# Samirez/Visual_odometry

Measured on AMD Instinct MI355X. Metric: frame-pairs/sec (1280x720, 2000 ORB feats), higher is better.
Workload: dtype u8+f32+f64; 1 GPU; seeded synthetic 1280x720 drone flight (256 distinct rendered views, closed loop), 2000 ORB features/frame, 8 levels = BASELINE config 2; chunk of 257 consecutive frames -> 256 pairs (k, k+1) per GPU per step, each frame detected once; detector=orb, distinct_rendered_frames=256, pair_stride=1, contexts_per_gpu=3, keypoint_order=cv2, poly_solver=fast, matcher=crosscheck, matcher_kernel=mfma_fp4, ransac=5-point, conf 0.99, 1 px, seed 2^64-1, <=1000 iters, parallelism=single GPU, pairs_ok_last_step=256

## Files before the change

visual_odometry_amd/csrc/geom_kernels.hip:

```cpp
#include "vo_internal.h"
#include "chain_common.h"
#include <float.h>

#define WAVE 64
#ifndef VO_DK_FAST_CAP
#define VO_DK_FAST_CAP 64
#endif
#ifndef VO_DK_ITERS
#define VO_DK_ITERS 300
#endif

__device__ __forceinline__ double vo_hypot(double a, double b)
{
    a = fabs(a); b = fabs(b);
    if (a < b) { double t = a; a = b; b = t; }
    if (a == 0) return 0;
    double r = b / a;
    return a * sqrt(1 + r * r);
}

template <int M, int N>
__device__ __forceinline__ void jacobi_svd(double* At, double* W, double* Vt)
{
    const double eps = DBL_EPSILON * 10;
// ... 98 lines not shown
{
    PolyTab t{};
    for (int i = 0; i < 4; i++)
        for (int j = 0; j < 4; j++) {
            int a = k_e1[i][0] + k_e1[j][0], b = k_e1[i][1] + k_e1[j][1], c = k_e1[i][2] + k_e1[j][2];
            int idx = -1;
            for (int m = 0; m < 10; m++) if (k_e2[m][0] == a && k_e2[m][1] == b && k_e2[m][2] == c) idx = m;
            t.t11[i][j] = idx;
        }
    for (int i = 0; i < 10; i++)
        for (int j = 0; j < 4; j++) {
            int a = k_e2[i][0] + k_e1[j][0], b = k_e2[i][1] + k_e1[j][1], c = k_e2[i][2] + k_e1[j][2];
            int idx = -1;
            for (int m = 0; m < 20; m++) if (k_e3[m][0] == a && k_e3[m][1] == b && k_e3[m][2] == c) idx = m;
            t.t21[i][j] = idx;
        }
    return t;
}

__device__ __forceinline__ void mul11_acc(const double* p, const double* q, double s, double* r)
{
    constexpr PolyTab T = make_poly_tab();
#pragma unroll
    for (int i = 0; i < 4; i++)
#pragma unroll
        for (int j = 0; j < 4; j++) r[T.t11[i][j]] += s * p[i] * q[j];
}

__device__ __forceinline__ void mul21_acc(const double* p, const double* q, double s, double* r)
{
    constexpr PolyTab T = make_poly_tab();
#pragma unroll
    for (int i = 0; i < 10; i++)
#pragma unroll
        for (int j = 0; j < 4; j++) r[T.t21[i][j]] += s * p[i] * q[j];
}

struct cplx { double re, im; };
__device__ __forceinline__ cplx cmul(cplx a, cplx b) { return {a.re * b.re - a.im * b.im, a.re * b.im + a.im * b.re}; }
__device__ __forceinline__ cplx cdiv(cplx a, cplx b)
{
    double t = 1. / (b.re * b.re + b.im * b.im);
    return {(a.re * b.re + a.im * b.im) * t, (-a.re * b.im + a.im * b.re) * t};
}

template <int NA, int NB>
__device__ __forceinline__ void conv(const double* a, const double* b, double* r)
{
#pragma unroll
    for (int i = 0; i <= NA + NB; i++) r[i] = 0;
#pragma unroll
    for (int i = 0; i <= NA; i++)
#pragma unroll
        for (int j = 0; j <= NB; j++) r[i + j] += a[i] * b[j];
}

template <int O>
__device__ __forceinline__ int quad_bcast(int v) { return __builtin_amdgcn_mov_dpp(v, O * 0x55, 0xf, 0xf, true); }
template <int O>
__device__ __forceinline__ double quad_bcast(double v)
{
    const int lo = quad_bcast<O>(__double2loint(v)), hi = quad_bcast<O>(__double2hiint(v));
    return __hiloint2double(hi, lo);
}
__device__ __forceinline__ double quad_bcast_from(int o, double v)
{
    switch (o) {
    case 0: return quad_bcast<0>(v);
    case 1: return quad_bcast<1>(v);
    case 2: return quad_bcast<2>(v);
    default: return quad_bcast<3>(v);
    }
}
__device__ __forceinline__ double sel4(int q, double a, double b, double c, double d) { return q == 0 ? a : q == 1 ? b : q == 2 ? c : d; }

__device__ __forceinline__ bool dk_exit(double max_diff, double max_mag, bool conv_all, bool early, double& prev, int& stall)
{
    if (max_diff <= 0 || (early && conv_all)) return true;
    const double small = 1e-7 * (1.0 + max_mag);
    if (early && max_diff < small * small) {
        if (max_diff > 0.25 * prev) { if (++stall >= 2) return true; }
        else stall = 0;
    }
    prev = max_diff;
    return false;
}

__device__ __forceinline__ void dk_iterate_quad(const double* c, double* rr, double* ri, bool early, int q)
{
    double prev = 1e300;
    int stall = 0;
    const int sweeps = early ? VO_DK_FAST_CAP : VO_DK_ITERS;
#pragma unroll 1
    for (int iter = 0; iter < sweeps; iter++) {
        bool conv_all = true;
        double max_diff = 0, max_mag = 0;
        double pr[3], pi[3], nr[3], ni[3], dr[3], di[3];
#pragma unroll
        for (int t = 0; t < 2; t++) {
            pr[t] = sel4(q, rr[4 * t], rr[4 * t + 1], rr[4 * t + 2], rr[4 * t + 3]);
            pi[t] = sel4(q, ri[4 * t], ri[4 * t + 1], ri[4 * t + 2], ri[4 * t + 3]);
        }
        pr[2] = (q & 1) ? rr[9] : rr[8]; pi[2] = (q & 1) ? ri[9] : ri[8];
#pragma unroll
        for (int t = 0; t < 3; t++) { nr[t] = c[10]; ni[t] = 0; dr[t] = c[10]; di[t] = 0; }
#pragma unroll
        for (int j = 0; j < 10; j++)
#pragma unroll
            for (int t = 0; t < 3; t++) {
                const cplx np = cmul({nr[t], ni[t]}, {pr[t], pi[t]});
                nr[t] = np.re + c[9 - j]; ni[t] = np.im;
            }
#pragma unroll
        for (int i = 0; i < 10; i++) {
            const int t = i >> 2, o = i & 3;
            cplx denom = {dr[t], di[t]};
#pragma unroll
            for (int j = i + 1; j < 10; j++) denom = cmul(denom, {pr[t] - rr[j], pi[t] - ri[j]});
            const bool coincident = q == o && !(fabs(denom.re) > 0) && !(fabs(denom.im) > 0);
            if (__any(coincident)) {
                if (coincident) {
                    denom = {c[10], 0};
#pragma unroll
                    for (int j = 0; j < 10; j++)
                        if (j != i) {
                            const cplx d = {rr[i] - rr[j], ri[i] - ri[j]};
                            if (d.re != 0 || d.im != 0) denom = cmul(denom, d);
                        }
                }
            }
            cplx num = cdiv({nr[t], ni[t]}, denom);
            num.re = quad_bcast_from(o, num.re); num.im = quad_bcast_from(o, num.im);
            rr[i] = rr[i] - num.re; ri[i] = ri[i] - num.im;
            const double ab2 = num.re * num.re + num.im * num.im;
            max_diff = fmax(max_diff, ab2);
            const double mag = fabs(rr[i]) + fabs(ri[i]);
            max_mag = fmax(max_mag, mag);
            const double lim = 4 * DBL_EPSILON * mag;
            conv_all &= ab2 <= lim * lim;
#pragma unroll
            for (int t2 = t; t2 < 3; t2++) {
                if (t2 == t && o == 3) continue;
                const cplx m = cmul({dr[t2], di[t2]}, {pr[t2] - rr[i], pi[t2] - ri[i]});
                const bool mine = t2 > t || q > o;
                dr[t2] = mine ? m.re : dr[t2]; di[t2] = mine ? m.im : di[t2];
            }
        }
        if (dk_exit(max_diff, max_mag, conv_all, early, prev, stall)) break;
    }
}

__device__ __forceinline__ void dk_iterate_low(const double* c, int n, double* rr, double* ri, bool early)
{
    double prev = 1e300;
    int stall = 0;
    const int sweeps = early ? VO_DK_FAST_CAP : VO_DK_ITERS;
#pragma unroll 1
    for (int iter = 0; iter < sweeps; iter++) {
        bool conv_all = true;
        double max_diff = 0, max_mag = 0;
#pragma unroll
        for (int i = 0; i < 10; i++) {
            if (i < n) {
                cplx p = {rr[i], ri[i]};
                double lead = c[10];
#pragma unroll
                for (int q = 1; q <= 10; q++) if (q == n) lead = c[q];
                cplx num = {lead, 0}, denom = {lead, 0};
#pragma unroll
                for (int j = 0; j < 10; j++) {
                    if (j < n) {
                        double cj = c[9 - j];
#pragma unroll
                        for (int q = 0; q < 10; q++) if (q == n - j - 1) cj = c[q];
                        cplx np = cmul(num, p);
                        num.re = np.re + cj; num.im = np.im;
                        if (j != i) {
                            cplx d = {p.re - rr[j], p.im - ri[j]};
                            if (d.re != 0 || d.im != 0) denom = cmul(denom, d);
                        }
                    }
                }
                num = cdiv(num, denom);
                rr[i] = p.re - num.re; ri[i] = p.im - num.im;
                const double ab2 = num.re * num.re + num.im * num.im;
                max_diff = fmax(max_diff, ab2);
                const double mag = fabs(rr[i]) + fabs(ri[i]);
                max_mag = fmax(max_mag, mag);
                const double lim = 4 * DBL_EPSILON * mag;
                conv_all &= ab2 <= lim * lim;
            }
        }
        if (dk_exit(max_diff, max_mag, conv_all, early, prev, stall)) break;
    }
}

#define FP_QUADS 16
typedef __attribute__((address_space(3))) double lds_double;
#define CMQ(r, j) cm[((r) * 5 + (j)) * 64 + lane]
#define CMK(r, k) cm[((r) * 5 + (k) % 5) * 64 + (lane & ~3) + (k) / 5]
__device__ __forceinline__ void quad_lds_sync()
{
    __builtin_amdgcn_fence(__ATOMIC_RELEASE, "wavefront");
    __builtin_amdgcn_wave_barrier();
    __builtin_amdgcn_fence(__ATOMIC_ACQUIRE, "wavefront");
}

__device__ __noinline__ int five_point_solve_quad(const double* x1, const double* x2, double* Eout, lds_double* cm, bool dk_early)
{
    const int lane = threadIdx.x & 63, q = lane & 3;
    double basis[36];
    {
        double A[9][5], V[5][9];
#pragma unroll
        for (int i = 0; i < 5; i++) {
            double u1 = x1[2 * i], v1 = x1[2 * i + 1], u2 = x2[2 * i], v2 = x2[2 * i + 1];
            A[0][i] = u2 * u1; A[1][i] = u2 * v1; A[2][i] = u2;
            A[3][i] = v2 * u1; A[4][i] = v2 * v1; A[5][i] = v2;
            A[6][i] = u1; A[7][i] = v1; A[8][i] = 1.0;
        }
        bool bad = false;
#pragma unroll
        for (int k = 0; k < 5; k++) {
            double nrm = 0;
#pragma unroll
            for (int r = k; r < 9; r++) nrm += A[r][k] * A[r][k];
            nrm = sqrt(nrm);
            bad |= nrm < 1e-300;
            double alpha = A[k][k] > 0 ? -nrm : nrm;
#pragma unroll
            for (int r = 0; r < 9; r++) V[k][r] = r < k ? 0.0 : A[r][k];
            V[k][k] -= alpha;
            double vn = 0;
#pragma unroll
            for (int r = k; r < 9; r++) vn += V[k][r] * V[k][r];
            vn = sqrt(vn);
            bad |= vn < 1e-300;
#pragma unroll
            for (int r = k; r < 9; r++) V[k][r] /= vn;
#pragma unroll
            for (int c = k; c < 5; c++) {
                double d = 0;
#pragma unroll
                for (int r = k; r < 9; r++) d += V[k][r] * A[r][c];
#pragma unroll
                for (int r = k; r < 9; r++) A[r][c] -= 2 * d * V[k][r];
            }
        }
        if (bad) return 0;
#pragma unroll
        for (int j = 0; j < 4; j++) {
            double e[9];
#pragma unroll
            for (int r = 0; r < 9; r++) e[r] = (r == 5 + j) ? 1.0 : 0.0;
#pragma unroll
            for (int k = 4; k >= 0; k--) {
                double d = 0;
#pragma unroll
                for (int r = k; r < 9; r++) d += V[k][r] * e[r];
#pragma unroll
                for (int r = k; r < 9; r++) e[r] -= 2 * d * V[k][r];
            }
#pragma unroll
            for (int r = 0; r < 9; r++) basis[j * 9 + r] = e[r];
        }
    }

    {
        double E[3][3][4];
#pragma unroll
        for (int r = 0; r < 3; r++)
#pragma unroll
            for (int c = 0; c < 3; c++)
#pragma unroll
                for (int k = 0; k < 4; k++) E[r][c][k] = basis[k * 9 + r * 3 + c];
        {
            double row[20];
#pragma unroll
            for (int i = 0; i < 20; i++) row[i] = 0;
#pragma unroll
            for (int c = 0; c < 3; c++) {
                const int c1 = (c + 1) % 3, c2 = (c + 2) % 3;
                double m[10];
#pragma unroll
                for (int i = 0; i < 10; i++) m[i] = 0;
                mul11_acc(E[1][c1], E[2][c2], 1.0, m);
                mul11_acc(E[1][c2], E[2][c1], -1.0, m);
                mul21_acc(m, E[0][c], 1.0, row);
            }
#pragma unroll
            for (int j = 0; j < 5; j++) CMQ(0, j) = sel4(q, row[j], row[5 + j], row[10 + j], row[15 + j]);
        }
        double L[3][3][10];
#pragma unroll
        for (int r = 0; r < 3; r++)
#pragma unroll
            for (int c = 0; c < 3; c++) {
#pragma unroll
                for (int i = 0; i < 10; i++) L[r][c][i] = 0;
#pragma unroll
                for (int k = 0; k < 3; k++) mul11_acc(E[r][k], E[c][k], 1.0, L[r][c]);
            }
        double tr[10];
#pragma unroll
        for (int i = 0; i < 10; i++) tr[i] = L[0][0][i] + L[1][1][i] + L[2][2][i];
#pragma unroll
        for (int r = 0; r < 3; r++)
#pragma unroll
            for (int i = 0; i < 10; i++) L[r][r][i] -= 0.5 * tr[i];
#pragma unroll
        for (int r = 0; r < 3; r++)
#pragma unroll
            for (int c = 0; c < 3; c++) {
                double row[20];
#pragma unroll
                for (int i = 0; i < 20; i++) row[i] = 0;
#pragma unroll
                for (int k = 0; k < 3; k++) mul21_acc(L[r][k], E[k][c], 1.0, row);
#pragma unroll
                for (int j = 0; j < 5; j++) CMQ(1 + r * 3 + c, j) = sel4(q, row[j], row[5 + j], row[10 + j], row[15 + j]);
            }
    }
    quad_lds_sync();

#pragma unroll 1
    for (int col = 0; col < 10; col++) {
        int piv = col;
        double best = fabs(CMK(col, col));
#pragma unroll 1
        for (int r = col + 1; r < 10; r++) { double v = fabs(CMK(r, col)); if (v > best) { best = v; piv = r; } }
        if (best < 1e-300) return 0;
        double prow[5], f[10];
        const double inv = 1.0 / CMK(piv, col);
        quad_lds_sync();
#pragma unroll
        for (int j = 0; j < 5; j++) {
            const double a = CMQ(piv, j), b = CMQ(col, j);
            prow[j] = a * inv;
            CMQ(piv, j) = b;
            CMQ(col, j) = prow[j];
        }
        quad_lds_sync();
#pragma unroll
        for (int r = 0; r < 10; r++) f[r] = CMK(r, col);
        quad_lds_sync();
#pragma unroll
        for (int r = 0; r < 10; r++) {
            if (r == col || f[r] == 0) continue;
#pragma unroll
            for (int j = 0; j < 5; j++) CMQ(r, j) -= f[r] * prow[j];
        }
        quad_lds_sync();
    }

    double Bx[3][4], By[3][4], Bc[3][5];
#pragma unroll
    for (int i = 0; i < 3; i++) {
        double r1[10], r2[10];
#pragma unroll
        for (int k = 0; k < 10; k++) { r1[k] = CMK(2 * i + 4, 10 + k); r2[k] = CMK(2 * i + 5, 10 + k); }
        Bx[i][3] = -r2[0]; Bx[i][2] = r1[0] - r2[1]; Bx[i][1] = r1[1] - r2[2]; Bx[i][0] = r1[2];
        By[i][3] = -r2[3]; By[i][2] = r1[3] - r2[4]; By[i][1] = r1[4] - r2[5]; By[i][0] = r1[5];
        Bc[i][4] = -r2[6]; Bc[i][3] = r1[6] - r2[7]; Bc[i][2] = r1[7] - r2[8]; Bc[i][1] = r1[8] - r2[9]; Bc[i][0] = r1[9];
    }
    double c[11];
    {
        double t1[8], t2[8], t3[11];
#pragma unroll
        for (int i = 0; i < 11; i++) c[i] = 0;
        conv<3, 4>(By[1], Bc[2], t1); conv<3, 4>(By[2], Bc[1], t2);
#pragma unroll
        for (int i = 0; i < 8; i++) t1[i] -= t2[i];
        conv<3, 7>(Bx[0], t1, t3);
#pragma unroll
        for (int i = 0; i < 11; i++) c[i] += t3[i];
        conv<3, 4>(Bx[1], Bc[2], t1); conv<3, 4>(Bx[2], Bc[1], t2);
#pragma unroll
        for (int i = 0; i < 8; i++) t1[i] -= t2[i];
        conv<3, 7>(By[0], t1, t3);
#pragma unroll
        for (int i = 0; i < 11; i++) c[i] -= t3[i];
        conv<3, 3>(Bx[1], By[2], t1); conv<3, 3>(Bx[2], By[1], t2);
#pragma unroll
        for (int i = 0; i < 7; i++) t1[i] -= t2[i];
        conv<4, 6>(Bc[0], t1, t3);
#pragma unroll
        for (int i = 0; i < 11; i++) c[i] += t3[i];
    }

    int n = 10;
    while (n > 1 && !(fabs(c[n]) > DBL_EPSILON)) n--;
    double rr[10], ri[10];
    {
        cplx p = {1, 0}, r = {1, 1};
#pragma unroll
        for (int i = 0; i < 10; i++) { rr[i] = p.re; ri[i] = p.im; p = cmul(p, r); }
    }
    if (n == 10) dk_iterate_quad(c, rr, ri, dk_early, q);
    else dk_iterate_low(c, n, rr, ri, dk_early);

    uint32_t real_mask = 0;
#pragma unroll
    for (int k = 0; k < 10; k++) {
        double zi = ri[k];
        if (fabs(zi) < 1e-100) zi = 0;
        if (k < n && !(fabs(zi) > 1e-10)) real_mask |= 1u << k;
    }
    const int nreal = __popc(real_mask);
    int count = 0;
#pragma unroll 1
    for (int m0 = 0; m0 < nreal; m0 += 4) {
        const int m = m0 + q;
        double zr = 0;
        {
            int ord = 0;
#pragma unroll
            for (int k = 0; k < 10; k++) {
                const bool set = (real_mask >> k) & 1;
                if (set && ord == m) zr = rr[k];
                ord += set;
            }
        }
        double en[9];
#pragma unroll
        for (int k = 0; k < 9; k++) en[k] = 0;
        int keep = 0;
        if (m < nreal) {
            double z1 = zr, z2 = z1 * z1, z3 = z2 * z1, z4 = z3 * z1;
            double bz[9], xy1[3];
#pragma unroll
            for (int j = 0; j < 3; j++) {
                bz[j * 3 + 0] = Bx[j][3] * z3 + Bx[j][2] * z2 + Bx[j][1] * z1 + Bx[j][0];
                bz[j * 3 + 1] = By[j][3] * z3 + By[j][2] * z2 + By[j][1] * z1 + By[j][0];
                bz[j * 3 + 2] = Bc[j][4] * z4 + Bc[j][3] * z3 + Bc[j][2] * z2 + Bc[j][1] * z1 + Bc[j][0];
            }
            solve_z<3>(bz, xy1);
            if (!(fabs(xy1[2]) < 1e-10)) {
                double x = xy1[0] / xy1[2], y = xy1[1] / xy1[2], nrm = 0, e[9];
#pragma unroll
                for (int k = 0; k < 9; k++) {
                    e[k] = basis[k] * x + basis[9 + k] * y + basis[18 + k] * z1 + basis[27 + k];
                    nrm += e[k] * e[k];
                }
                nrm = sqrt(nrm);
#pragma unroll
                for (int k = 0; k < 9; k++) en[k] = e[k] / nrm;
                keep = 1;
            }
        }
#define FP_STORE_MODEL(o)                                                                             \
        if (quad_bcast<o>(keep)) {                                                                    \
            double w[9];                                                                              \
            _Pragma("unroll") for (int k = 0; k < 9; k++) w[k] = quad_bcast<o>(en[k]);                \
            double* dst = Eout + count * 9;                                                           \
            dst[q] = sel4(q, w[0], w[1], w[2], w[3]);                                                 \
            dst[4 + q] = sel4(q, w[4], w[5], w[6], w[7]);                                             \
            dst[8] = w[8];                                                                            \
            count++;                                                                                  \
        }
        FP_STORE_MODEL(0) FP_STORE_MODEL(1) FP_STORE_MODEL(2) FP_STORE_MODEL(3)
#undef FP_STORE_MODEL
    }
    return count;
}

__device__ __forceinline__ uint32_t rng_next(uint64_t& state)
{
    state = (uint64_t)(uint32_t)state * 4164903690ULL + (uint32_t)(state >> 32);
    return (uint32_t)state;
}

__device__ int ransac_update_num_iters(double p, double ep, int model_points, int max_iters)
{
    p = fmax(p, 0.); p = fmin(p, 1.);
    ep = fmax(ep, 0.); ep = fmin(ep, 1.);
    double num = fmax(1. - p, DBL_MIN);
    double denom = 1. - pow(1. - ep, (double)model_points);
    if (denom < DBL_MIN) return 0;
    num = log(num);
    denom = log(denom);
    return (denom >= 0 || -num >= max_iters * (-denom)) ? max_iters : __double2int_rn(num / denom);
}

__device__ __forceinline__ float sampson_err(const double* E, double u1, double v1, double u2, double v2)
{
    double Ex0 = E[0] * u1 + E[1] * v1 + E[2], Ex1 = E[3] * u1 + E[4] * v1 + E[5], Ex2 = E[6] * u1 + E[7] * v1 + E[8];
    double Et0 = E[0] * u2 + E[3] * v2 + E[6], Et1 = E[1] * u2 + E[4] * v2 + E[7];
    double d = u2 * Ex0 + v2 * Ex1 + Ex2;
    return (float)(d * d / (Ex0 * Ex0 + Ex1 * Ex1 + Et0 * Et0 + Et1 * Et1));
}

__device__ __forceinline__ int count_inliers(const double* E, const double* x1, const double* x2, int M, float t,
                                             int lane, int stride, int first, uint8_t* mask_out)
{
    int good = 0;
    for (int base = first; base < M; base += stride) {
        const int i = base + lane;
        bool f = false;
        if (i < M) {
            f = sampson_err(E, x1[2 * i], x1[2 * i + 1], x2[2 * i], x2[2 * i + 1]) <= t;
            if (mask_out) mask_out[i] = f ? 1 : 0;
        }
        good += __popcll(__ballot(f));
    }
    return good;
}

#define RS_STREAM 512
#define RS_SCORE_G 4
#ifndef RS_WAVES
#define RS_WAVES 4
#endif
#ifndef RS_SOLVERS
#define RS_SOLVERS 4
#endif
#define RS_ROUND (FP_QUADS * RS_SOLVERS)
#define RS_THREADS (64 * RS_WAVES)
static_assert(RS_SOLVERS >= 1 && RS_SOLVERS <= RS_WAVES && RS_ROUND <= 64, "the sampler and the model list hold at most 64 samples per round");

struct RansacShared {
    double cm[200 * RS_ROUND];
    uint32_t stream[RS_STREAM];
    int sub[64][5];
    int nm[64];
    int off[65];
    uint8_t eh[640];
    int cnt[RS_WAVES * RS_SCORE_G];
    int used;
};

__global__ __launch_bounds__(RS_THREADS, 1) void k_ransac(PairBuf pb, int kp_cap, RansacParams rp, const uint32_t* rng_tab, int rng_n)
{
    extern __shared__ __attribute__((aligned(16))) unsigned char s_dyn[];
    RansacShared& sh = *(RansacShared*)s_dyn;
    const int p = blockIdx.x, tid = threadIdx.x, lane = tid & 63, wave = tid >> 6;
    const int M = pb.m_count[p];
    const double* x1 = pb.xn1 + (size_t)p * kp_cap * 2;
    const double* x2 = pb.xn2 + (size_t)p * kp_cap * 2;
    uint8_t* mask = pb.mask + (size_t)p * kp_cap;
    vo_pair_result* res = pb.res + p;

    if (M < 5) {
        if (tid == 0) { res->status = VO_ERR_TOO_FEW; res->n_inl = 0; res->ransac_iters = 0; }
        for (int i = tid; i < M; i += RS_THREADS) mask[i] = 0;
        return;
    }
    const double threshold = rp.thresh_px / ((rp.K[0] + rp.K[4]) / 2);
    const float t = (float)(threshold * threshold);

    if (M == 5) {
        if (tid < 4) {
            double* models = pb.models + (size_t)p * 64 * 90;
            const int nm = five_point_solve_quad(x1, x2, models, (lds_double*)sh.cm, rp.dk_early != 0);
            __threadfence_block();
            if (tid == 0) {
                for (int k = 0; k < 9; k++) res->E[k] = nm > 0 ? models[k] : 0.0;
                res->status = nm > 0 ? VO_OK : VO_ERR_NO_MODEL;
                res->n_inl = nm > 0 ? 5 : 0;
                res->reserved = nm;
                res->ransac_iters = 0;
            }
        }
        if (tid < 5) mask[tid] = 1;
        return;
    }

    int niters = rp.max_iters > 1 ? rp.max_iters : 1;
    int max_good = 0, iters_done = 0, pos = 0;
    double bestE[9];
#pragma unroll
    for (int k = 0; k < 9; k++) bestE[k] = 0;

#ifdef VO_EXP_TIMING
    long long tA = clock64(), tB = 0, tC = 0, tD = 0, tE = 0;
#endif
    double* gmodels = pb.models + (size_t)p * 64 * 90;
    for (int r0 = 0; r0 < niters; r0 += RS_ROUND) {
        const int nh = min(RS_ROUND, niters - r0);
        for (int i = tid; i < RS_STREAM; i += RS_THREADS) sh.stream[i] = pos + i < rng_n ? rng_tab[pos + i] % (uint32_t)M : 0u;
        __syncthreads();
        if (wave == 0) {
            int start = 5 * lane, used = 5;
            for (;;) {
                int idx[5];
                used = 0;
                if (lane < nh) {
#pragma unroll
                    for (int i = 0; i < 5; i++) {
                        int v; bool dup;
                        do {
                            const int at = start + used;
                            if (at < RS_STREAM && pos + at < rng_n) v = (int)sh.stream[at];
                            else {
                                uint64_t st = rp.seed ? rp.seed : 0xffffffffULL;
                                uint32_t x = 0;
                                if (pos + at < rng_n) x = rng_tab[pos + at];
                                else { for (int q = 0; q <= pos + at; q++) x = rng_next(st); }
                                v = (int)(x % (uint32_t)M);
                            }
                            used++;
                            dup = false;
#pragma unroll
                            for (int k = 0; k < 5; k++) dup |= k < i && idx[k] == v;
                        } while (dup);
                        idx[i] = v;
                    }
#pragma unroll
                    for (int i = 0; i < 5; i++) sh.sub[lane][i] = idx[i];
                }
                int inc = used;
#pragma unroll
                for (int d = 1; d < 64; d <<= 1) { const int o = __shfl_up(inc, d, 64); if (lane >= d) inc += o; }
                const int true_start = inc - used;
                const bool moved = lane < nh && true_start != start;
                start = true_start;
                if (lane == 63) sh.used = inc;
                if (!__any(moved)) break;
            }
        }
        __syncthreads();
        pos += sh.used;
#ifdef VO_EXP_TIMING
        if (r0 == 0) tB = clock64();
#endif
        if (wave < RS_SOLVERS) {
            const int h = wave * FP_QUADS + (lane >> 2);
            if (h < nh) {
                double s1[10], s2[10];
#pragma unroll
                for (int i = 0; i < 5; i++) {
                    const int v = sh.sub[h][i];
                    s1[2 * i] = x1[2 * v]; s1[2 * i + 1] = x1[2 * v + 1];
                    s2[2 * i] = x2[2 * v]; s2[2 * i + 1] = x2[2 * v + 1];
                }
                const int nm = five_point_solve_quad(s1, s2, gmodels + h * 90, (lds_double*)sh.cm + wave * (200 * FP_QUADS), rp.dk_early != 0);
                if ((lane & 3) == 0) sh.nm[h] = nm;
            }
        }
        __syncthreads();
        if (wave == 0) {
            const int nm = lane < nh ? sh.nm[lane] : 0;
            int inc = nm;
#pragma unroll
            for (int d = 1; d < 64; d <<= 1) { int v = __shfl_up(inc, d, 64); if (lane >= d) inc += v; }
            sh.off[lane] = inc - nm;
            if (lane == 63) sh.off[64] = inc;
            for (int m = 0; m < nm; m++) sh.eh[inc - nm + m] = (uint8_t)lane;
        }
        __syncthreads();
#ifdef VO_EXP_TIMING
        if (r0 == 0) tC = clock64();
#endif
        const int T = sh.off[64];
        bool done = false;
        int last_h = -1;
        for (int b0 = 0; b0 < T && !done; b0 += RS_WAVES * RS_SCORE_G) {
            {
                double E[RS_SCORE_G][9];
                int ne = 0;
#pragma unroll
                for (int gq = 0; gq < RS_SCORE_G; gq++) {
                    const int e = b0 + gq * RS_WAVES + wave;
                    const int ee = e < T ? e : (b0 + wave < T ? b0 + wave : 0);
                    const int h = sh.eh[ee], m = ee - sh.off[h];
#pragma unroll
                    for (int k = 0; k < 9; k++) E[gq][k] = gmodels[h * 90 + m * 9 + k];
                    ne += e < T;
                }
                if (ne > 0) {
                    int good[RS_SCORE_G];
#pragma unroll
                    for (int gq = 0; gq < RS_SCORE_G; gq++) good[gq] = 0;
                    for (int base = 0; base < M; base += 64) {
                        const int i = base + lane;
                        const bool in = i < M;
                        const double u1 = in ? x1[2 * i] : 0.0, v1 = in ? x1[2 * i + 1] : 0.0, u2 = in ? x2[2 * i] : 0.0, v2 = in ? x2[2 * i + 1] : 0.0;
#pragma unroll
                        for (int gq = 0; gq < RS_SCORE_G; gq++)
                            good[gq] += (int)__popcll(__ballot(in && sampson_err(E[gq], u1, v1, u2, v2) <= t));
                    }
                    if (lane == 0) {
#pragma unroll
                        for (int gq = 0; gq < RS_SCORE_G; gq++) sh.cnt[gq * RS_WAVES + wave] = good[gq];
                    }
                }
            }
            __syncthreads();
            for (int q = 0; q < RS_WAVES * RS_SCORE_G; q++) {
                const int e2 = b0 + q;
                if (e2 >= T) break;
                const int h = sh.eh[e2];
                if (h != last_h) {
                    if (r0 + h >= niters) { done = true; break; }
                    last_h = h;
                    iters_done = r0 + h + 1;
                }
                const int good = sh.cnt[q];
                if (good > max(max_good, 4)) {
                    const int m = e2 - sh.off[h];
#pragma unroll
                    for (int k = 0; k < 9; k++) bestE[k] = gmodels[h * 90 + m * 9 + k];
                    max_good = good;
                    niters = ransac_update_num_iters(rp.prob, (double)(M - good) / M, 5, niters);
                }
            }
            __syncthreads();
        }
        if (!done) iters_done = min(r0 + nh, niters);
        __syncthreads();
#ifdef VO_EXP_TIMING
        if (r0 == 0) tD = clock64();
#endif
    }

    if (max_good > 0) {
        count_inliers(bestE, x1, x2, M, t, tid, RS_THREADS, 0, mask);
        if (tid == 0) {
#pragma unroll
            for (int k = 0; k < 9; k++) res->E[k] = bestE[k];
            res->n_inl = max_good; res->status = VO_OK; res->ransac_iters = iters_done; res->reserved = 1;
#ifdef VO_EXP_TIMING
            tE = clock64();
            res->n_kp1 = (int)(tB - tA); res->n_kp2 = (int)(tC - tB); res->n_match = (int)(tD - tC); res->n_good = (int)(tE - tD); res->reserved = iters_done;
#endif
        }
    } else {
        for (int i = tid; i < M; i += RS_THREADS) mask[i] = 0;
        if (tid == 0) { res->n_inl = 0; res->status = VO_ERR_NO_MODEL; res->ransac_iters = iters_done; res->reserved = 0; }
    }
}

void launch_ransac(hipStream_t s, PairBuf pb, int kp_cap, int P, RansacParams rp, const uint32_t* rng_tab, int rng_n)
{
    static bool attr = false;
    if (!attr) { (void)hipFuncSetAttribute((const void*)k_ransac, hipFuncAttributeMaxDynamicSharedMemorySize, (int)sizeof(RansacShared)); attr = true; }
    hipLaunchKernelGGL(k_ransac, dim3(P), dim3(RS_THREADS), sizeof(RansacShared), s, pb, kp_cap, rp, rng_tab, rng_n);
}

__device__ __forceinline__ void triangulate_one(const double* P1, const double* P2, double x1, double y1,
                                                double x2, double y2, double* X)
{
    double A[16];
#pragma unroll
    for (int k = 0; k < 4; k++) {
        A[0 * 4 + k] = x1 * P1[8 + k] - P1[k];
        A[1 * 4 + k] = y1 * P1[8 + k] - P1[4 + k];
        A[2 * 4 + k] = x2 * P2[8 + k] - P2[k];
        A[3 * 4 + k] = y2 * P2[8 + k] - P2[4 + k];
    }
    solve_z<4>(A, X);
}

__global__ void k_triangulate_raw(const double* P1g, const double* P2g, const double* x1, const double* x2,
                                  int M, double* X)
{
    int i = blockIdx.x * blockDim.x + threadIdx.x;
    if (i >= M) return;
    double P1[12], P2[12], q[4];
#pragma unroll
    for (int k = 0; k < 12; k++) { P1[k] = P1g[k]; P2[k] = P2g[k]; }
    triangulate_one(P1, P2, x1[i], x1[M + i], x2[i], x2[M + i], q);
#pragma unroll
    for (int k = 0; k < 4; k++) X[(size_t)k * M + i] = q[k];
}

void launch_triangulate_raw(hipStream_t s, const double* P1, const double* P2, const double* x1, const double* x2,
                            int M, double* X)
{
    if (M <= 0) return;
    hipLaunchKernelGGL(k_triangulate_raw, dim3((M + 63) / 64), dim3(64), 0, s, P1, P2, x1, x2, M, X);
}

__global__ void k_triangulate_pairs(PairBuf pb, int kp_cap, RansacParams rp)
{
    const int p = blockIdx.y;
    const vo_pair_result* res = pb.res + p;
    if (res->status != VO_OK) return;
    int i = blockIdx.x * blockDim.x + threadIdx.x;
    if (i >= res->n_inl) return;
    const double* R = res->R; const double* t = res->t; const double* K = rp.K;
    double T[12], P[12], P0[12];
#pragma unroll
    for (int r = 0; r < 3; r++) {
#pragma unroll
        for (int c = 0; c < 3; c++) T[r * 4 + c] = R[c * 3 + r];
        T[r * 4 + 3] = -(R[0 * 3 + r] * t[0] + R[1 * 3 + r] * t[1] + R[2 * 3 + r] * t[2]);
    }
#pragma unroll
// ... 76 lines not shown
{
    double Q[4];
    triangulate_one(P0, P, a[0], a[1], b[0], b[1], Q);
    const double w = Q[2] * Q[3];
    const double q0 = Q[0] / Q[3], q1 = Q[1] / Q[3], q2 = Q[2] / Q[3], q3 = Q[3] / Q[3];
    const double z = P[8] * q0 + P[9] * q1 + P[10] * q2 + P[11] * q3;
    pos = w > 0 && q2 < dist && z > 0 && z < dist;
    neg = w < 0 && -q2 < dist && -z > 0 && -z < dist;
}

__global__ __launch_bounds__(256) void k_pose_prepare(PairBuf pb, int kp_cap)
{
    __shared__ int s_w[4];
    const int p = blockIdx.x, tid = threadIdx.x, lane = tid & 63, wave = tid >> 6;
    vo_pair_result* res = pb.res + p;
    PoseState* ps = pb.pose_state + p;
    if (res->status != VO_OK) {
        if (tid == 0) { res->n_good = 0; ps->active = 0; }
        return;
    }
    if (res->reserved != 1) {
        __syncthreads();
        if (tid == 0) { res->status = VO_ERR_AMBIGUOUS; res->n_good = 0; ps->active = 0; }
        return;
    }
    const int M = pb.m_count[p];
    const size_t base2 = (size_t)p * kp_cap * 2;
    const uint8_t* mask = pb.mask + (size_t)p * kp_cap;
    double* in1 = pb.in1 + base2; double* in2 = pb.in2 + base2;
    double* ip1 = pb.ipx1 + base2; double* ip2 = pb.ipx2 + base2;
    int ninl = 0;
    for (int b = 0; b < M; b += 256) {
        const int i = b + tid;
        const bool f = i < M && mask[i] != 0;
        const unsigned long long bal = __ballot(f);
        __syncthreads();
        if (lane == 0) s_w[wave] = __popcll(bal);
        __syncthreads();
        int off = 0, tot = 0;
#pragma unroll
        for (int w = 0; w < 4; w++) { const int c = s_w[w]; if (w < wave) off += c; tot += c; }
        if (f) {
            const int pos = ninl + off + __popcll(bal & ((1ULL << lane) - 1));
            in1[2 * pos] = pb.xn1[base2 + 2 * i]; in1[2 * pos + 1] = pb.xn1[base2 + 2 * i + 1];
            in2[2 * pos] = pb.xn2[base2 + 2 * i]; in2[2 * pos + 1] = pb.xn2[base2 + 2 * i + 1];
            ip1[2 * pos] = pb.px1[base2 + 2 * i]; ip1[2 * pos + 1] = pb.px1[base2 + 2 * i + 1];
            ip2[2 * pos] = pb.px2[base2 + 2 * i]; ip2[2 * pos + 1] = pb.px2[base2 + 2 * i + 1];
        }
        ninl += tot;
    }
    if (tid < 64) {
        double E[9], R1[9], R2[9], tt[3];
#pragma unroll
        for (int k = 0; k < 9; k++) E[k] = res->E[k];
        decompose_essential(E, R1, R2, tt);
        if (tid == 0) {
#pragma unroll
            for (int k = 0; k < 9; k++) { ps->R1[k] = R1[k]; ps->R2[k] = R2[k]; }
#pragma unroll
            for (int k = 0; k < 3; k++) ps->t[k] = tt[k];
#pragma unroll
            for (int k = 0; k < 4; k++) ps->good[k] = 0;
            ps->ninl = ninl; ps->active = 1;
        }
    }
}

__device__ __forceinline__ void pose_candidate(const PoseState* ps, int c, double* P)
{
    const double* Rc = c ? ps->R2 : ps->R1;
#pragma unroll
    for (int r = 0; r < 3; r++) {
#pragma unroll
        for (int k = 0; k < 3; k++) P[r * 4 + k] = Rc[r * 3 + k];
        P[r * 4 + 3] = ps->t[r];
    }
}

__global__ __launch_bounds__(256) void k_pose(PairBuf pb, int kp_cap, RansacParams rp)
{
    const int p = blockIdx.x, blk = blockIdx.y, c = blockIdx.z, lane = threadIdx.x & 63;
    PoseState* ps = pb.pose_state + p;
    if (!ps->active) return;
    const int ninl = ps->ninl, i = blk * 256 + threadIdx.x;
    if (blk * 256 >= ninl) return;
    const size_t base2 = (size_t)p * kp_cap * 2;
    const double* in1 = pb.in1 + base2; const double* in2 = pb.in2 + base2;
    const double P0[12] = {1, 0, 0, 0, 0, 1, 0, 0, 0, 0, 1, 0};
    double P[12];
    pose_candidate(ps, c, P);
    bool mp = false, mn = false;
    if (i < ninl) cheirality2(P0, P, in1 + 2 * i, in2 + 2 * i, rp.dist_thresh, mp, mn);
    const int gp = __popcll(__ballot(mp)), gn = __popcll(__ballot(mn));
    if (lane == 0 && gp) atomicAdd(&ps->good[c], gp);
    if (lane == 0 && gn) atomicAdd(&ps->good[c + 2], gn);
}

__global__ __launch_bounds__(256) void k_pose_finish(PairBuf pb, int kp_cap, RansacParams rp)
{
    const int p = blockIdx.x;
    const PoseState* ps = pb.pose_state + p;
    if (!ps->active) return;
    vo_pair_result* res = pb.res + p;
    const int ninl = ps->ninl;
    const int g0 = ps->good[0], g1 = ps->good[1], g2 = ps->good[2], g3 = ps->good[3];
    int best;
    if (g0 >= g1 && g0 >= g2 && g0 >= g3) best = 0;
    else if (g1 >= g0 && g1 >= g2 && g1 >= g3) best = 1;
    else if (g2 >= g0 && g2 >= g1 && g2 >= g3) best = 2;
    else best = 3;
    if (pb.pose_mask) {
        const size_t base2 = (size_t)p * kp_cap * 2;
        const double* in1 = pb.in1 + base2; const double* in2 = pb.in2 + base2;
        const double P0[12] = {1, 0, 0, 0, 0, 1, 0, 0, 0, 0, 1, 0};
        double P[12];
        pose_candidate(ps, best & 1, P);
        uint8_t* pm = pb.pose_mask + (size_t)p * kp_cap;
        for (int i = threadIdx.x; i < ninl; i += blockDim.x) {
            bool mp, mn;
            cheirality2(P0, P, in1 + 2 * i, in2 + 2 * i, rp.dist_thresh, mp, mn);
            pm[i] = (best >= 2 ? mn : mp) ? 255 : 0;
        }
    }
    if (threadIdx.x == 0) {
        const double* Rb = (best & 1) ? ps->R2 : ps->R1;
#pragma unroll
        for (int k = 0; k < 9; k++) res->R[k] = Rb[k];
#pragma unroll
        for (int k = 0; k < 3; k++) res->t[k] = best >= 2 ? -ps->t[k] : ps->t[k];
        res->n_good = best == 0 ? g0 : best == 1 ? g1 : best == 2 ? g2 : g3;
        res->n_inl = ninl;
    }
}

void launch_pose(hipStream_t s, PairBuf pb, int kp_cap, int P, RansacParams rp)
{
    hipLaunchKernelGGL(k_pose_prepare, dim3(P), dim3(256), 0, s, pb, kp_cap);
    hipLaunchKernelGGL(k_pose, dim3(P, (kp_cap + 255) / 256, 2), dim3(256), 0, s, pb, kp_cap, rp);
    hipLaunchKernelGGL(k_pose_finish, dim3(P), dim3(pb.pose_mask ? 256 : 64), 0, s, pb, kp_cap, rp);
}

__global__ __launch_bounds__(64) void k_five_point_raw(const double* x1, const double* x2, double* E, int* nm, int dk_early)
{
    extern __shared__ __attribute__((aligned(16))) unsigned char s_dyn[];
    if (threadIdx.x < 4 && blockIdx.x == 0) {
        const int n = five_point_solve_quad(x1, x2, E, (lds_double*)s_dyn, dk_early != 0);
        if (threadIdx.x == 0) *nm = n;
    }
}

void launch_five_point_raw(hipStream_t s, const double* x1, const double* x2, double* E, int* nm, int dk_early)
{
    static bool attr = false;
    if (!attr) { (void)hipFuncSetAttribute((const void*)k_five_point_raw, hipFuncAttributeMaxDynamicSharedMemorySize, (int)(200 * FP_QUADS * sizeof(double))); attr = true; }
    hipLaunchKernelGGL(k_five_point_raw, dim3(1), dim3(64), 200 * FP_QUADS * sizeof(double), s, x1, x2, E, nm, dk_early);
}

__global__ void k_reprojection(const double* poses, int ncam, const double* points, int npt, const int* obs_cam,
                               const int* obs_pt, const double* obs_xy, int nobs, const double* Kd, double threshold,
                               double* sqerr, uint8_t* keep, int* bad)
{
    const int i = blockIdx.x * blockDim.x + threadIdx.x;
    if (i >= nobs) return;
    const int ci = obs_cam[i], pi = obs_pt[i];
    if (ci < 0 || ci >= ncam || pi < 0 || pi >= npt) { atomicOr(bad, 1); sqerr[i] = 0; keep[i] = 0; return; }
    const double e = reprojection_sqerr_one(poses + 16 * (size_t)ci, points + 3 * (size_t)pi, Kd, obs_xy[2 * i], obs_xy[2 * i + 1]);
    sqerr[i] = e;
    keep[i] = e < threshold ? 1 : 0;
}

void launch_reprojection(hipStream_t s, const double* poses, int ncam, const double* points, int npt, const int* obs_cam,
                         const int* obs_pt, const double* obs_xy, int nobs, const double* Kd, double threshold,
                         double* sqerr, uint8_t* keep, int* bad)
{
    if (nobs <= 0) return;
    hipLaunchKernelGGL(k_reprojection, dim3((nobs + 255) / 256), dim3(256), 0, s, poses, ncam, points, npt, obs_cam, obs_pt,
                       obs_xy, nobs, Kd, threshold, sqerr, keep, bad);
}

__global__ void k_track_link(const int* pair_frames, const int* match_off, const int* mq, const int* mt, int P, int cap,
                             unsigned long long* parent)
{
    const int p = blockIdx.y;
    const int n = match_off[p + 1] - match_off[p];
    const int i = blockIdx.x * blockDim.x + threadIdx.x;
    if (i >= n) return;
    const int f1 = pair_frames[2 * p], f2 = pair_frames[2 * p + 1];
    const int q = mq[match_off[p] + i], t = mt[match_off[p] + i];
    const unsigned long long v = ((unsigned long long)(p + 1) << 40) | ((unsigned long long)(unsigned)f1 << 20) | (unsigned)q;
    atomicMax(&parent[(size_t)f2 * cap + t], v);
}

__global__ void k_track_roots(const unsigned long long* parent, int F, int cap, int* root_frame, int* root_idx, int* hops, int* bad)
{
    const int i = blockIdx.x * blockDim.x + threadIdx.x, f = blockIdx.y;
    if (i >= cap) return;
    int cf = f, ci = i, n = 0;
    for (;;) {
        const unsigned long long v = parent[(size_t)cf * cap + ci];
        if (v == 0) break;
        cf = (int)((v >> 20) & 0xfffffu); ci = (int)(v & 0xfffffu);
        if (++n > F) { atomicOr(bad, 1); break; }
    }
    root_frame[(size_t)f * cap + i] = cf; root_idx[(size_t)f * cap + i] = ci; hops[(size_t)f * cap + i] = n;
}

void launch_tracks(hipStream_t s, const int* pair_frames, const int* match_off, const int* mq, const int* mt, int P, int max_m,
                   int F, int cap, unsigned long long* parent, int* root_frame, int* root_idx, int* hops, int* bad)
{
    if (P > 0 && max_m > 0)
        hipLaunchKernelGGL(k_track_link, dim3((max_m + 255) / 256, P), dim3(256), 0, s, pair_frames, match_off, mq, mt, P, cap, parent);
    hipLaunchKernelGGL(k_track_roots, dim3((cap + 255) / 256, F), dim3(256), 0, s, parent, F, cap, root_frame, root_idx, hops, bad);
}


__global__ void k_chain_link(PairBuf pb, int kp_cap, ChainBuf cb)
{
    const int p = blockIdx.y, i = blockIdx.x * blockDim.x + threadIdx.x;
    if (pb.res[p].status != VO_OK || i >= pb.m_count[p] || !pb.mask[(size_t)p * kp_cap + i]) return;
    const int f1 = pb.slots[2 * p], f2 = pb.slots[2 * p + 1];
    const int q = pb.m_q[(size_t)p * kp_cap + i], t = pb.m_t[(size_t)p * kp_cap + i];
    const unsigned long long v = ((unsigned long long)(p + 1) << 40) | ((unsigned long long)(unsigned)f1 << 20) | (unsigned)q;
    atomicMax(&cb.parent[chain_key(f2, t, kp_cap)], v);
}

void launch_chain_link(hipStream_t s, PairBuf pb, int kp_cap, int P, ChainBuf cb)
{
    hipLaunchKernelGGL(k_chain_link, dim3((kp_cap + 255) / 256, P), dim3(256), 0, s, pb, kp_cap, cb);
}

__global__ __launch_bounds__(256) void k_chain_init(PairBuf pb, int kp_cap, ChainBuf cb) { chain_init_wg(pb, kp_cap, cb); }

__global__ __launch_bounds__(256) void k_chain_init_seqs(PairBuf pb, int kp_cap, const SlamSeq* __restrict__ seqs)
{
    const SlamSeq& q = seqs[blockIdx.x];
    chain_init_wg(chain_pairs_from(pb, q.first, kp_cap), kp_cap, q.cb);
}

void launch_chain_init_seqs(hipStream_t s, PairBuf pb, int kp_cap, const SlamSeq* seqs, int S)
{
    hipLaunchKernelGGL(k_chain_init_seqs, dim3(S), dim3(256), 0, s, pb, kp_cap, seqs);
}

void launch_chain_init(hipStream_t s, PairBuf pb, int kp_cap, ChainBuf cb)
{
    hipLaunchKernelGGL(k_chain_init, dim3(1), dim3(256), 0, s, pb, kp_cap, cb);
}

__device__ __forceinline__ void chain_gather_wg(PairBuf pb, int kp_cap, int p, int F, ChainBuf cb)
{
    __shared__ int s_w[4];
    __shared__ int s_base;
    const int tid = threadIdx.x, lane = tid & 63, wave = tid >> 6;
    const vo_pair_result& r = pb.res[p];
    const int f1 = pb.slots[2 * p], f2 = pb.slots[2 * p + 1];
    if (cb.rs.st) {
        const bool lost = !cb.alive[0];
        if (r.status != VO_OK || lost) {
            if (tid == 0) {
                cb.off[0] = cb.obj0; cb.off[1] = cb.obj0; cb.n_corr[p] = 0;
                if (r.status != VO_OK) {
                    cb.status[p] = r.status; cb.alive[0] = 0; cb.rs.st[SEG_INIT] = 0;
                    if (cb.rs.st[SEG_CAUSE] == 0) cb.rs.st[SEG_CAUSE] = r.status;
                } else cb.rs.st[SEG_INIT] = 1;
            }
            return;
        }
        if (tid == 0) cb.rs.st[SEG_INIT] = 0;
    }
    const bool ok = cb.alive[0] && r.status == VO_OK && cb.cam_ok[f1];
    if (!ok) {
        if (tid == 0) {
            cb.off[0] = cb.obj0; cb.off[1] = cb.obj0; cb.n_corr[p] = 0;
            cb.status[p] = !cb.alive[0] ? VO_ERR_NOT_CONFIGURED : r.status != VO_OK ? r.status : VO_ERR_INVALID;
            cb.alive[0] = 0;
            if (cb.rs.st && cb.rs.st[SEG_CAUSE] == 0) cb.rs.st[SEG_CAUSE] = cb.status[p];
        }
        return;
    }
    if (tid == 0) s_base = 0;
    const int M = pb.m_count[p];
    const uint8_t* mask = pb.mask + (size_t)p * kp_cap;
    const double* px2 = pb.px2 + (size_t)p * kp_cap * 2;
    for (int b = 0; b < M; b += 256) {
        const int i = b + tid;
        bool take = false; size_t key = 0;
        if (i < M && mask[i]) {
            int rf = f2, ri = pb.m_t[(size_t)p * kp_cap + i];
            chain_root(cb.parent, kp_cap, F, rf, ri);
            key = chain_key(rf, ri, kp_cap);
            take = cb.in_map[key] != 0;
        }
        const unsigned long long bal = __ballot(take);
        __syncthreads();
        if (lane == 0) s_w[wave] = __popcll(bal);
        __syncthreads();
        int off = 0, tot = 0;
        for (int w = 0; w < 4; w++) { const int c = s_w[w]; if (w < wave) off += c; tot += c; }
        if (take) {
            const int pos = s_base + off + (int)__popcll(bal & ((1ULL << lane) - 1));
            for (int d = 0; d < 3; d++) cb.obj[3 * pos + d] = cb.map_pt[3 * key + d];
            cb.img[2 * pos] = px2[2 * i]; cb.img[2 * pos + 1] = px2[2 * i + 1];
        }
        __syncthreads();
        if (tid == 0) s_base += tot;
        __syncthreads();
    }
    if (tid == 0) { cb.off[0] = cb.obj0; cb.off[1] = cb.obj0 + s_base; cb.n_corr[p] = s_base; }
// ... 88 lines not shown
```

Measured before the change: 101,300 frame-pairs/s.

## Keep five-point elimination matrix in registers, park basis in LDS, raise RANSAC occupancy

Moves the 10x20 Gauss-Jordan elimination in the five-point solver out of LDS and into per-lane registers, using quad broadcasts and compile-time unrolled pivot steps instead of LDS round trips and wave barriers. The null-space basis and the B polynomial coefficients are parked in a much smaller LDS region so registers are freed before root finding. This shrinks the shared memory the RANSAC kernel needs and sets waves-per-EU to 2 so more blocks can be resident. It also pre-shifts the polynomial coefficients once in the Durand-Kerner loop instead of selecting them every iteration, and inlines the solver. The cost is much higher register pressure, with a risk of spills, and more select instructions for the pivot swaps.

```diff
diff --git a/visual_odometry_amd/csrc/geom_kernels.hip b/visual_odometry_amd/csrc/geom_kernels.hip
--- a/visual_odometry_amd/csrc/geom_kernels.hip
+++ b/visual_odometry_amd/csrc/geom_kernels.hip
@@ -274,6 +274,16 @@
 
 __device__ __forceinline__ void dk_iterate_low(const double* c, int n, double* rr, double* ri, bool early)
 {
+    double s[11];
+#pragma unroll
+    for (int k = 0; k <= 10; k++) s[k] = c[k];
+#pragma unroll
+    for (int step = 0; step < 9; step++) {
+        const bool move = step < 10 - n;
+#pragma unroll
+        for (int k = 10; k >= 1; k--) s[k] = move ? s[k - 1] : s[k];
+        s[0] = move ? 0.0 : s[0];
+    }
     double prev = 1e300;
     int stall = 0;
     const int sweeps = early ? VO_DK_FAST_CAP : VO_DK_ITERS;
@@ -285,16 +295,12 @@
         for (int i = 0; i < 10; i++) {
             if (i < n) {
                 cplx p = {rr[i], ri[i]};
-                double lead = c[10];
-#pragma unroll
-                for (int q = 1; q <= 10; q++) if (q == n) lead = c[q];
+                const double lead = s[10];
                 cplx num = {lead, 0}, denom = {lead, 0};
 #pragma unroll
                 for (int j = 0; j < 10; j++) {
                     if (j < n) {
-                        double cj = c[9 - j];
-#pragma unroll
-                        for (int q = 0; q < 10; q++) if (q == n - j - 1) cj = c[q];
+                        const double cj = s[9 - j];
                         cplx np = cmul(num, p);
                         num.re = np.re + cj; num.im = np.im;
                         if (j != i) {
@@ -317,20 +323,53 @@
     }
 }
 
+template <int COL>
+__device__ __forceinline__ bool elim_step(double (&cmr)[10][5])
+{
+    double colv[10];
+#pragma unroll
+    for (int r = 0; r < 10; r++) colv[r] = quad_bcast<COL / 5>(cmr[r][COL % 5]);
+    int piv = COL;
+    double best = fabs(colv[COL]), pv = colv[COL];
+#pragma unroll
+    for (int r = COL + 1; r < 10; r++) { const double v = fabs(colv[r]); if (v > best) { best = v; piv = r; pv = colv[r]; } }
+    if (best < 1e-300) return false;
+    double prow[5];
+    const double inv = 1.0 / pv;
+#pragma unroll
+    for (int j = 0; j < 5; j++) {
+        const double b = cmr[COL][j];
+        double a = b;
+#pragma unroll
+        for (int r = COL + 1; r < 10; r++) a = piv == r ? cmr[r][j] : a;
+        prow[j] = a * inv;
+#pragma unroll
+        for (int r = COL + 1; r < 10; r++) cmr[r][j] = piv == r ? b : cmr[r][j];
+        cmr[COL][j] = prow[j];
+    }
+#pragma unroll
+    for (int r = 0; r < 10; r++) {
+        if (r == COL) continue;
+        const double f = (r > COL && piv == r) ? colv[COL] : colv[r];
+        const bool skip = f == 0;
+#pragma unroll
+        for (int j = 0; j < 5; j++) {
+            const double v = cmr[r][j] - f * prow[j];
+            cmr[r][j] = skip ? cmr[r][j] : v;
+        }
+    }
+    return true;
+}
+
 #define FP_QUADS 16
+#define FP_PARK 75
 typedef __attribute__((address_space(3))) double lds_double;
-#define CMQ(r, j) cm[((r) * 5 + (j)) * 64 + lane]
-#define CMK(r, k) cm[((r) * 5 + (k) % 5) * 64 + (lane & ~3) + (k) / 5]
-__device__ __forceinline__ void quad_lds_sync()
-{
-    __builtin_amdgcn_fence(__ATOMIC_RELEASE, "wavefront");
-    __builtin_amdgcn_wave_barrier();
-    __builtin_amdgcn_fence(__ATOMIC_ACQUIRE, "wavefront");
-}
-
-__device__ __noinline__ int five_point_solve_quad(const double* x1, const double* x2, double* Eout, lds_double* cm, bool dk_early)
+#define PARK(i) park[(i) * FP_QUADS + (lane >> 2)]
+
+__device__ __forceinline__ int five_point_solve_quad(const double* x1, const double* x2, double* Eout, lds_double* park, bool dk_early)
 {
     const int lane = threadIdx.x & 63, q = lane & 3;
+    double cmr[10][5];
     double basis[36];
     {
         double A[9][5], V[5][9];
@@ -411,76 +450,64 @@
                 mul21_acc(m, E[0][c], 1.0, row);
             }
 #pragma unroll
-            for (int j = 0; j < 5; j++) CMQ(0, j) = sel4(q, row[j], row[5 + j], row[10 + j], row[15 + j]);
-        }
-        double L[3][3][10];
+            for (int j = 0; j < 5; j++) cmr[0][j] = sel4(q, row[j], row[5 + j], row[10 + j], row[15 + j]);
+        }
+        double D[3][10], tr[10];
+#pragma unroll
+        for (int r = 0; r < 3; r++) {
+#pragma unroll
+            for (int i = 0; i < 10; i++) D[r][i] = 0;
+#pragma unroll
+            for (int k = 0; k < 3; k++) mul11_acc(E[r][k], E[r][k], 1.0, D[r]);
+        }
+#pragma unroll
+        for (int i = 0; i < 10; i++) tr[i] = D[0][i] + D[1][i] + D[2][i];
 #pragma unroll
         for (int r = 0; r < 3; r++)
 #pragma unroll
+            for (int i = 0; i < 10; i++) D[r][i] -= 0.5 * tr[i];
+#pragma unroll
+        for (int r = 0; r < 3; r++) {
+            double L[3][10];
+#pragma unroll
             for (int c = 0; c < 3; c++) {
-#pragma unroll
-                for (int i = 0; i < 10; i++) L[r][c][i] = 0;
-#pragma unroll
-                for (int k = 0; k < 3; k++) mul11_acc(E[r][k], E[c][k], 1.0, L[r][c]);
-            }
-        double tr[10];
-#pragma unroll
-        for (int i = 0; i < 10; i++) tr[i] = L[0][0][i] + L[1][1][i] + L[2][2][i];
-#pragma unroll
-        for (int r = 0; r < 3; r++)
-#pragma unroll
-            for (int i = 0; i < 10; i++) L[r][r][i] -= 0.5 * tr[i];
-#pragma unroll
-        for (int r = 0; r < 3; r++)
+                if (c == r) {
+#pragma unroll
+                    for (int i = 0; i < 10; i++) L[c][i] = D[r][i];
+                } else {
+#pragma unroll
+                    for (int i = 0; i < 10; i++) L[c][i] = 0;
+#pragma unroll
+                    for (int k = 0; k < 3; k++) mul11_acc(E[r][k], E[c][k], 1.0, L[c]);
+                }
+            }
 #pragma unroll
             for (int c = 0; c < 3; c++) {
                 double row[20];
 #pragma unroll
                 for (int i = 0; i < 20; i++) row[i] = 0;
 #pragma unroll
-                for (int k = 0; k < 3; k++) mul21_acc(L[r][k], E[k][c], 1.0, row);
-#pragma unroll
-                for (int j = 0; j < 5; j++) CMQ(1 + r * 3 + c, j) = sel4(q, row[j], row[5 + j], row[10 + j], row[15 + j]);
-            }
-    }
-    quad_lds_sync();
-
-#pragma unroll 1
-    for (int col = 0; col < 10; col++) {
-        int piv = col;
-        double best = fabs(CMK(col, col));
-#pragma unroll 1
-        for (int r = col + 1; r < 10; r++) { double v = fabs(CMK(r, col)); if (v > best) { best = v; piv = r; } }
-        if (best < 1e-300) return 0;
-        double prow[5], f[10];
-        const double inv = 1.0 / CMK(piv, col);
-        quad_lds_sync();
-#pragma unroll
-        for (int j = 0; j < 5; j++) {
-            const double a = CMQ(piv, j), b = CMQ(col, j);
-            prow[j] = a * inv;
-            CMQ(piv, j) = b;
-            CMQ(col, j) = prow[j];
-        }
-        quad_lds_sync();
-#pragma unroll
-        for (int r = 0; r < 10; r++) f[r] = CMK(r, col);
-        quad_lds_sync();
-#pragma unroll
-        for (int r = 0; r < 10; r++) {
-            if (r == col || f[r] == 0) continue;
-#pragma unroll
-            for (int j = 0; j < 5; j++) CMQ(r, j) -= f[r] * prow[j];
-        }
-        quad_lds_sync();
-    }
+                for (int k = 0; k < 3; k++) mul21_acc(L[k], E[k][c], 1.0, row);
+#pragma unroll
+                for (int j = 0; j < 5; j++) cmr[1 + r * 3 + c][j] = sel4(q, row[j], row[5 + j], row[10 + j], row[15 + j]);
+            }
+        }
+    }
+#pragma unroll
+    for (int i = 0; i < 36; i++) PARK(i) = basis[i];
+
+    if (!elim_step<0>(cmr) || !elim_step<1>(cmr) || !elim_step<2>(cmr) || !elim_step<3>(cmr) || !elim_step<4>(cmr) ||
+        !elim_step<5>(cmr) || !elim_step<6>(cmr) || !elim_step<7>(cmr) || !elim_step<8>(cmr) || !elim_step<9>(cmr)) return 0;
 
     double Bx[3][4], By[3][4], Bc[3][5];
 #pragma unroll
     for (int i = 0; i < 3; i++) {
         double r1[10], r2[10];
 #pragma unroll
-        for (int k = 0; k < 10; k++) { r1[k] = CMK(2 * i + 4, 10 + k); r2[k] = CMK(2 * i + 5, 10 + k); }
+        for (int k = 0; k < 10; k++) {
+            r1[k] = quad_bcast_from(2 + k / 5, cmr[2 * i + 4][k % 5]);
+            r2[k] = quad_bcast_from(2 + k / 5, cmr[2 * i + 5][k % 5]);
+        }
         Bx[i][3] = -r2[0]; Bx[i][2] = r1[0] - r2[1]; Bx[i][1] = r1[1] - r2[2]; Bx[i][0] = r1[2];
         By[i][3] = -r2[3]; By[i][2] = r1[3] - r2[4]; By[i][1] = r1[4] - r2[5]; By[i][0] = r1[5];
         Bc[i][4] = -r2[6]; Bc[i][3] = r1[6] - r2[7]; Bc[i][2] = r1[7] - r2[8]; Bc[i][1] = r1[8] - r2[9]; Bc[i][0] = r1[9];
@@ -510,8 +537,18 @@
         for (int i = 0; i < 11; i++) c[i] += t3[i];
     }
 
+#pragma unroll
+    for (int i = 0; i < 3; i++) {
+#pragma unroll
+        for (int k = 0; k < 4; k++) { PARK(36 + i * 4 + k) = Bx[i][k]; PARK(48 + i * 4 + k) = By[i][k]; }
+#pragma unroll
+        for (int k = 0; k < 5; k++) PARK(60 + i * 5 + k) = Bc[i][k];
+    }
+    __asm__ volatile("" ::: "memory");
+
     int n = 10;
-    while (n > 1 && !(fabs(c[n]) > DBL_EPSILON)) n--;
+#pragma unroll
+    for (int k = 10; k > 1; k--) if (n == k && !(fabs(c[k]) > DBL_EPSILON)) n = k - 1;
     double rr[10], ri[10];
     {
         cplx p = {1, 0}, r = {1, 1};
@@ -552,16 +589,17 @@
             double bz[9], xy1[3];
 #pragma unroll
             for (int j = 0; j < 3; j++) {
-                bz[j * 3 + 0] = Bx[j][3] * z3 + Bx[j][2] * z2 + Bx[j][1] * z1 + Bx[j][0];
-                bz[j * 3 + 1] = By[j][3] * z3 + By[j][2] * z2 + By[j][1] * z1 + By[j][0];
-                bz[j * 3 + 2] = Bc[j][4] * z4 + Bc[j][3] * z3 + Bc[j][2] * z2 + Bc[j][1] * z1 + Bc[j][0];
+                const int bx = 36 + j * 4, by = 48 + j * 4, bc = 60 + j * 5;
+                bz[j * 3 + 0] = PARK(bx + 3) * z3 + PARK(bx + 2) * z2 + PARK(bx + 1) * z1 + PARK(bx);
+                bz[j * 3 + 1] = PARK(by + 3) * z3 + PARK(by + 2) * z2 + PARK(by + 1) * z1 + PARK(by);
+                bz[j * 3 + 2] = PARK(bc + 4) * z4 + PARK(bc + 3) * z3 + PARK(bc + 2) * z2 + PARK(bc + 1) * z1 + PARK(bc);
             }
             solve_z<3>(bz, xy1);
             if (!(fabs(xy1[2]) < 1e-10)) {
                 double x = xy1[0] / xy1[2], y = xy1[1] / xy1[2], nrm = 0, e[9];
 #pragma unroll
                 for (int k = 0; k < 9; k++) {
-                    e[k] = basis[k] * x + basis[9 + k] * y + basis[18 + k] * z1 + basis[27 + k];
+                    e[k] = PARK(k) * x + PARK(9 + k) * y + PARK(18 + k) * z1 + PARK(27 + k);
                     nrm += e[k] * e[k];
                 }
                 nrm = sqrt(nrm);
@@ -636,12 +674,15 @@
 #ifndef RS_SOLVERS
 #define RS_SOLVERS 4
 #endif
+#ifndef RS_OCC
+#define RS_OCC 2
+#endif
 #define RS_ROUND (FP_QUADS * RS_SOLVERS)
 #define RS_THREADS (64 * RS_WAVES)
 static_assert(RS_SOLVERS >= 1 && RS_SOLVERS <= RS_WAVES && RS_ROUND <= 64, "the sampler and the model list hold at most 64 samples per round");
 
 struct RansacShared {
-    double cm[200 * RS_ROUND];
+    double park[FP_PARK * RS_ROUND];
     uint32_t stream[RS_STREAM];
     int sub[64][5];
     int nm[64];
@@ -651,7 +692,7 @@
     int used;
 };
 
-__global__ __launch_bounds__(RS_THREADS, 1) void k_ransac(PairBuf pb, int kp_cap, RansacParams rp, const uint32_t* rng_tab, int rng_n)
+__global__ __launch_bounds__(RS_THREADS) __attribute__((amdgpu_waves_per_eu(RS_OCC, RS_OCC))) void k_ransac(PairBuf pb, int kp_cap, RansacParams rp, const uint32_t* rng_tab, int rng_n)
 {
     extern __shared__ __attribute__((aligned(16))) unsigned char s_dyn[];
     RansacShared& sh = *(RansacShared*)s_dyn;
@@ -673,7 +714,7 @@
     if (M == 5) {
         if (tid < 4) {
             double* models = pb.models + (size_t)p * 64 * 90;
-            const int nm = five_point_solve_quad(x1, x2, models, (lds_double*)sh.cm, rp.dk_early != 0);
+            const int nm = five_point_solve_quad(x1, x2, models, (lds_double*)sh.park, rp.dk_early != 0);
             __threadfence_block();
             if (tid == 0) {
                 for (int k = 0; k < 9; k++) res->E[k] = nm > 0 ? models[k] : 0.0;
@@ -755,7 +796,7 @@
                     s1[2 * i] = x1[2 * v]; s1[2 * i + 1] = x1[2 * v + 1];
                     s2[2 * i] = x2[2 * v]; s2[2 * i + 1] = x2[2 * v + 1];
                 }
-                const int nm = five_point_solve_quad(s1, s2, gmodels + h * 90, (lds_double*)sh.cm + wave * (200 * FP_QUADS), rp.dk_early != 0);
+                const int nm = five_point_solve_quad(s1, s2, gmodels + h * 90, (lds_double*)sh.park + wave * (FP_PARK * FP_QUADS), rp.dk_early != 0);
                 if ((lane & 3) == 0) sh.nm[h] = nm;
             }
         }
@@ -1138,8 +1179,8 @@
 void launch_five_point_raw(hipStream_t s, const double* x1, const double* x2, double* E, int* nm, int dk_early)
 {
     static bool attr = false;
-    if (!attr) { (void)hipFuncSetAttribute((const void*)k_five_point_raw, hipFuncAttributeMaxDynamicSharedMemorySize, (int)(200 * FP_QUADS * sizeof(double))); attr = true; }
-    hipLaunchKernelGGL(k_five_point_raw, dim3(1), dim3(64), 200 * FP_QUADS * sizeof(double), s, x1, x2, E, nm, dk_early);
+    if (!attr) { (void)hipFuncSetAttribute((const void*)k_five_point_raw, hipFuncAttributeMaxDynamicSharedMemorySize, (int)(FP_PARK * FP_QUADS * sizeof(double))); attr = true; }
+    hipLaunchKernelGGL(k_five_point_raw, dim3(1), dim3(64), FP_PARK * FP_QUADS * sizeof(double), s, x1, x2, E, nm, dk_early);
 }
 
 __global__ void k_reprojection(const double* poses, int ncam, const double* points, int npt, const int* obs_cam,
```

Result: faster. 105,200 frame-pairs/s (median of 6 runs) (+3.8%).
